# wsakobe/CylinderTag

Measured on AMD Instinct MI355X. Metric: frames/sec detect() 1920x1080, higher is better.
Workload: dtype u8; 1 GPU; synthetic 1920x1080 random-stripe frames, 4096 per step over 1 GPU(s), 4 planted CTag_2f12c markers each, detect(img,5,true,5), inputs resident in HBM; frames_per_gpu=4096, chunk=4096, parallelism=frames sharded, dp1, gather=none (1 GPU)

## Files before the change

### cylindertag_amd/csrc/ctag_api.hip

```cpp
#include <hip/hip_runtime.h>

#include <algorithm>
#include <climits>
#include <cmath>
#include <cstdio>
#include <cstdlib>
#include <cstring>
#include <fstream>
#include <map>
#include <mutex>
#include <new>
#include <string>
#include <type_traits>
#include <vector>

#include "../../include/ctag.h"
#include "ctag_internal.h"

using namespace ctag;

#define HIP_TRY(expr)                                                                                   \
    do {                                                                                                \
        hipError_t e__ = (expr);                                                                        \
        if (e__ != hipSuccess) {                                                                        \
// ... 262 lines not shown
    put(W.xmin, pool);
    put(W.ymin, pool);
    put(W.xmax, pool);
    put(W.ymax, pool);
    put(W.key, pool);
    put(W.pool_tile, pool);
    put(W.member_head, pool);
    put(W.member_next, pool);
    put(W.ncand, F * 4);
    put(W.nroots, F * 4);
    put(W.cand, F * CC * sizeof(Candidate));
    put(W.quads, F * CC * sizeof(QuadOut));
    put(W.line_count, F * 4);
    put(W.clp_used, F * 4);
    put(W.line_long, F * 4);
    put(W.cl_pool, F * (size_t)W.cl_cap * 4 + 16);
    put(W.line_desc, F * LC * sizeof(LineDesc));
    put(W.line_sorted, F * LC * 4);
    put(W.line_fit, F * LC * 16);
    put(W.cand_aux, F * CC * sizeof(CandAux));
    put(W.npacks, F * 8);
    put(W.packs, F * CC * 4);
    put(W.pack_order, F * CC * 4);
    put(W.welsch_rs, std::min<size_t>(F, kLatencyFrames) * kLatLines * 20 * 6 * 4);
    put(W.quad_derived, F * kQuadStride * 48);
    put(W.quad_index, F * kQuadStride * 4);
    put(W.nquads, F * 4);
    put(W.nfeat, F * 4);
    put(W.status, F * 4);
    put(W.feat0, F * CTAG_MAX_FEATURES * sizeof(FeatureDev));
    put(W.feat1, F * CTAG_MAX_FEATURES * sizeof(FeatureDev));
    put(W.feat2, F * CTAG_MAX_FEATURES * sizeof(FeatureDev));
    put(W.premarkers, F * sizeof(ctag_frame_result));
    put(W.frame_long, F * 4);
    put(W.rz_xofs, (size_t)g.hcols * 4);
    put(W.rz_alpha, (size_t)g.hcols * 8);
    put(W.rz_yofs, (size_t)g.hrows * 4);
    put(W.rz_beta, (size_t)g.hrows * 8);
    return off;
}

static int ensure_workspace(ctag_handle* h, ctag_handle::WsSlot& S, int rows, int cols, int tw, int frames, bool big, bool need_n0) {
    auto refresh = [&](Workspace& W) {
        const Caps c = make_caps(make_geom(rows, cols, tw, h->params.area_max_fraction), h->params, big);
        W.g = make_geom(rows, cols, tw, h->params.area_max_fraction);
        W.g.pool_cap = c.pool_cap;
// ... 1025 lines not shown
```

### cylindertag_amd/csrc/ctag_internal.h

```cpp
#pragma once
#include <hip/hip_runtime.h>
#include <stddef.h>
#include <stdint.h>

#include <vector>

#include "../../include/ctag_types.h"

struct ctag_handle;
struct ctag_camera;
struct ctag_pose_rec;
struct ctag_rig_pose_rec;
struct ctag_mv_pose_rec;
struct ctag_camera_set;

namespace ctag {
template <class T>
struct DevBuf {
    T* p = nullptr;
    size_t cap = 0;
    DevBuf() = default;
    DevBuf(const DevBuf&) = delete;
    DevBuf& operator=(const DevBuf&) = delete;
    ~DevBuf() { release(); }
// ... 152 lines not shown
    int32_t* key = nullptr;
    int32_t* pool_tile = nullptr;
    int32_t* member_head = nullptr;
    int32_t* member_next = nullptr;
    int32_t* ncand = nullptr;
    int32_t* nroots = nullptr;
    int cand_cap = 0;
    int line_cap = 0;
    uint32_t cl_cap = 0;
    bool big = false;
    Candidate* cand = nullptr;
    QuadOut* quads = nullptr;
    int32_t* line_count = nullptr;
    int32_t* clp_used = nullptr;
    uint32_t* cl_pool = nullptr;
    LineDesc* line_desc = nullptr;
    int32_t* line_sorted = nullptr;
    int32_t* line_long = nullptr;
    float* line_fit = nullptr;
    CandAux* cand_aux = nullptr;
    int32_t* npacks = nullptr;
    uint32_t* packs = nullptr;
    uint32_t* pack_order = nullptr;
    float* welsch_rs = nullptr;
    const uint8_t* pick_table = nullptr;
    const uint16_t* pick_table16 = nullptr;
    hipStream_t aux_stream = nullptr;
    hipEvent_t ev_fork = nullptr, ev_join = nullptr;
    KParams kp{};
    void* quad_derived = nullptr;
    int32_t* quad_index = nullptr;
    int32_t* nquads = nullptr;
    int32_t* nfeat = nullptr;
    int32_t* status = nullptr;
    FeatureDev* feat0 = nullptr;
    FeatureDev* feat1 = nullptr;
    FeatureDev* feat2 = nullptr;
    ctag_frame_result* premarkers = nullptr;
    double* refine_n0 = nullptr;
    int32_t* frame_long = nullptr;
    int32_t* rz_xofs = nullptr;
    int16_t* rz_alpha = nullptr;
    int32_t* rz_yofs = nullptr;
    int16_t* rz_beta = nullptr;
    void* base = nullptr;
    size_t bytes = 0;
// ... 161 lines not shown
```

### cylindertag_amd/csrc/k_quad.hip

```cpp
#include "ctag_internal.h"
#include "ctag_math.h"
#include "ctag_wave.h"
#include <cstdio>
#include <type_traits>
#include <cstdlib>

namespace ctag {

struct QuadPtrs {
    const uint16_t* labels;
    const int32_t* tile_base;
    const int32_t* root_of;
    const int32_t* ncand;
    const Candidate* cand;
    QuadOut* quads;
    uint32_t* frame_flags;
    int32_t* line_count;
    int32_t* clp_used;
    uint32_t* cl_pool;
    LineDesc* line_desc;
    int32_t* line_sorted;
    int32_t* line_long;
    float* line_fit;
    CandAux* cand_aux;
    const uint8_t* pick_table;
    const uint16_t* pick_table16;
    const int32_t* pool_tile;
    const int32_t* member_head;
    const int32_t* member_next;
    int32_t* npacks;
    uint32_t* packs;
    uint32_t* pack_order;
    unsigned long long* stamps;
    float thr_line, thr_expand, rac;
    int c2_far, c2_near;
    int cand_cap, line_cap;
    uint32_t cl_cap;
    float expand_eps;
    const uint64_t* mask;
    int mask_words;
};
static QuadPtrs quad_ptrs(const ChunkPlan& pl, const Workspace& ws, unsigned long long* stamps) {
    QuadPtrs P{};
    P.labels = ws.labels, P.tile_base = ws.tile_base, P.root_of = ws.root_of, P.ncand = ws.ncand, P.cand = ws.cand, P.quads = ws.quads, P.frame_flags = ws.frame_flags;
    P.line_count = ws.line_count, P.clp_used = ws.clp_used, P.cl_pool = ws.cl_pool, P.line_desc = ws.line_desc, P.line_sorted = ws.line_sorted, P.line_long = ws.line_long;
    P.line_fit = ws.line_fit, P.cand_aux = ws.cand_aux, P.pick_table = ws.pick_table, P.pick_table16 = ws.pick_table16;
    P.pool_tile = ws.pool_tile, P.member_head = ws.member_head, P.member_next = ws.member_next;
    P.npacks = ws.npacks, P.packs = ws.packs, P.pack_order = ws.pack_order, P.stamps = stamps;
    P.thr_line = ws.kp.thr_line, P.thr_expand = ws.kp.thr_expand, P.rac = ws.kp.rac, P.c2_far = ws.kp.c2_far, P.c2_near = ws.kp.c2_near, P.expand_eps = ws.kp.expand_eps;
    P.cand_cap = ws.cand_cap, P.line_cap = ws.line_cap, P.cl_cap = ws.cl_cap;
    P.mask = pl.fused ? reinterpret_cast<const uint64_t*>(ws.half) : nullptr, P.mask_words = ws.g.hcols >> 6;
    return P;
}

__device__ __forceinline__ uint32_t pack_xy(int x, int y) { return (uint32_t)x | ((uint32_t)y << 16); }
__device__ __forceinline__ int ux(uint32_t p) { return (int)(p & 0xffffu); }
__device__ __forceinline__ int uy(uint32_t p) { return (int)(p >> 16); }

__device__ __forceinline__ void moments_to_line(double x, double y, double x2, double y2, double xy, double w, float* line) {
    const ctm::Recip64 W = ctm::recip64(w);
    x = ctm::div64(x, W);
    y = ctm::div64(y, W);
    x2 = ctm::div64(x2, W);
    y2 = ctm::div64(y2, W);
    xy = ctm::div64(xy, W);
    const double dx2 = x2 - x * x, dy2 = y2 - y * y, dxy = xy - x * y;
    const float t = (float)ctm::atan2_64(2 * dxy, dx2 - dy2) / 2;
    double sn, cs;
    ctm::sincos64(t, &sn, &cs);
    line[0] = (float)cs;
    line[1] = (float)sn;
// ... 217 lines not shown
    (void)welsch_rounds<WS, COUNT>(pts, n, EPS, line, err, 0, 30, false, wc, min(n, kWCap), trips);
    restart_store(res, rstride, line, err);
}

#ifndef CTAG_PACK_WORDS
#define CTAG_PACK_WORDS 5120
#endif
#ifndef CTAG_PACK_WAVES
#define CTAG_PACK_WAVES 2
#endif
constexpr int kPackWords = CTAG_PACK_WORDS;
#ifndef CTAG_PACK_WAVES_P2
#define CTAG_PACK_WAVES_P2 4
#endif
constexpr int kPackWordsSmall = 2560, kPackWavesSmall = 4, kPackWavesSmallP2 = CTAG_PACK_WAVES_P2;
constexpr int kUnwind = 8;
constexpr int kWaveWords = 8192;
constexpr int kWaveWordsMax = 36864;
__host__ __device__ __forceinline__ int pack_points(int w, int h) { return min(2 * (w + h), w * h) + 1; }
__host__ __device__ __forceinline__ int pack_need(int w, int h) {
    const int C = pack_points(w, h);
    return ((w + 1) & ~1) + 2 * h + 2 * C + 4;
}
constexpr int kScanWords = 2048;
__host__ __device__ __forceinline__ int scan_need(int w, int h) { return w + 3 * h + 4; }
constexpr int kMaskScanWords = 512, kMaskScanWordsLarge = 2048;
__host__ __device__ __forceinline__ int mask_scan_need(int w, int h) { return h * ((w + 31) / 32 + 1); }
__host__ __device__ __forceinline__ bool pack_big(int x_min, int w, int h, int big_points, int pack_words, int scan_words = 0) {
    (void)x_min;
    return pack_need(w, h) > pack_words || pack_points(w, h) > big_points || (scan_words > 0 && scan_need(w, h) > scan_words) ||
           (scan_words < 0 && mask_scan_need(w, h) > -scan_words);
}

struct CornerPre {
    float x, y, dis, ang;
};

__global__ __launch_bounds__(1024) void k_pack(QuadPtrs P, int nframes, int max_per_pack, int big_points, int pack_words, int scan_words) {
    __shared__ int s_key[kLdsCand + 2];
    __shared__ int s_need[kLdsCand];
    __shared__ uint16_t s_ord[kLdsCand];
    const int frame = blockIdx.x;
    if (frame >= nframes) return;
    const int tid = threadIdx.x, nt = blockDim.x;
    const int nc = min(P.ncand[frame], P.cand_cap);
    const Candidate* cand = P.cand + (size_t)frame * P.cand_cap;
    uint32_t* order = P.pack_order + (size_t)frame * P.cand_cap;
    uint32_t* packs = P.packs + (size_t)frame * P.cand_cap;
    auto key_of = [&](const Candidate& c) {
        const int w = c.x_max - c.x_min + 1, h = c.y_max - c.y_min + 1;
        return pack_big(c.x_min, w, h, big_points, pack_words, scan_words) ? -1 : pack_points(w, h);
    };
    auto build_packs = [&](int npacked, auto need_of) {
        int np = 0, first = -1, cnt = 0, words = 0;
        for (int r0 = 0; r0 < npacked; r0 += 64) {
            const int r = r0 + tid;
            const int need = r < npacked ? need_of(r) : 0;
            const int m = min(64, npacked - r0);
            for (int k = 0; k < m; k++) {
                const int nk = __builtin_amdgcn_readlane(need, k);
                if (cnt > 0 && (cnt == max_per_pack || words + nk > pack_words)) {
                    if (tid == 0) packs[np] = (uint32_t)first | ((uint32_t)cnt << 24);
                    np++;
                    cnt = 0;
                    words = 0;
                }
                if (cnt == 0) first = r0 + k;
                cnt++;
                words += nk;
            }
        }
        if (cnt > 0) {
            if (tid == 0) packs[np] = (uint32_t)first | ((uint32_t)cnt << 24);
            np++;
        }
        return np;
    };
    auto slot_prefix = [&](int npacked, auto ci_of) {
        int base = 0;
        for (int r0 = 0; r0 < npacked; r0 += 64) {
            const int r = r0 + tid;
            int v = 0, ci = 0;
            if (r < npacked) {
                ci = ci_of(r);
                const Candidate c = cand[ci];
                v = pack_points(c.x_max - c.x_min + 1, c.y_max - c.y_min + 1) + 64;
            }
            int incl = v;
#pragma unroll
            for (int d = 1; d < 64; d <<= 1) {
                const int t = __shfl_up(incl, d, 64);
                if (tid >= d) incl += t;
            }
            if (r < npacked) P.cand_aux[(size_t)frame * P.cand_cap + ci].line0 = base + incl - v;
            base += __shfl(incl, 63, 64);
        }
        if (tid == 0) P.clp_used[frame] = base;
    };
    if (nc > kLdsCand) {
        constexpr int kB = kLdsCand;
        auto bucket_of = [&](int key) { return key < 0 ? kB : kB - 1 - min(key, kB - 1); };
        for (int b = tid; b <= kB; b += nt) s_key[b] = 0;
        __syncthreads();
        for (int i = tid; i < nc; i += nt) atomicAdd(&s_key[bucket_of(key_of(cand[i]))], 1);
        __syncthreads();
        if (tid == 0) {
            int run = 0;
            for (int b = 0; b <= kB; b++) {
                const int v = s_key[b];
                s_key[b] = run;
                run += v;
            }
            s_key[kB + 1] = run;
        }
        __syncthreads();
        const int first_big = s_key[kB];
        __syncthreads();
        for (int i = tid; i < nc; i += nt) order[atomicAdd(&s_key[bucket_of(key_of(cand[i]))], 1)] = (uint32_t)i;
        __syncthreads();
        if (tid >= 64) return;
        const int np = build_packs(first_big, [&](int r) {
            const Candidate c = cand[order[r]];
            return pack_need(c.x_max - c.x_min + 1, c.y_max - c.y_min + 1);
        });
        if (tid == 0) {
            P.npacks[2 * frame] = np;
            P.npacks[2 * frame + 1] = nc - first_big;
        }
        if (scan_words < 0) slot_prefix(first_big, [&](int r) { return (int)order[r]; });
        return;
    }
    for (int i = tid; i < nc; i += nt) {
        const Candidate c = cand[i];
        const int w = c.x_max - c.x_min + 1, h = c.y_max - c.y_min + 1;
        s_key[i] = key_of(c);
        s_need[i] = pack_need(w, h);
    }
    if (tid == 0) s_key[kLdsCand] = 0;
    __syncthreads();
    for (int i = tid; i < nc; i += nt) {
        const int ki = s_key[i];
        int rank = 0;
        for (int j = 0; j < nc; j++) {
            const int kj = s_key[j];
            rank += (kj > ki || (kj == ki && j < i)) ? 1 : 0;
        }
        s_ord[rank] = (uint16_t)i;
        if (ki < 0) atomicAdd(&s_key[kLdsCand], 1);
    }
    __syncthreads();
    for (int i = tid; i < nc; i += nt) order[i] = s_ord[i];
    if (tid >= 64) return;
    const int nbig = s_key[kLdsCand];
    const int np = build_packs(nc - nbig, [&](int r) { return s_need[s_ord[r]]; });
    if (tid == 0) {
        P.npacks[2 * frame] = np;
        P.npacks[2 * frame + 1] = nbig;
    }
    if (scan_words < 0) slot_prefix(nc - nbig, [&](int r) { return (int)s_ord[r]; });
}


#ifndef CTAG_EXPAND_INLINE
#define CTAG_EXPAND_INLINE __forceinline__
#endif
struct ALine {
    double c, s, x, y;
    bool ok;
};
__device__ __forceinline__ ALine approx_line(long long sx, long long sy, long long sxx, long long syy, long long sxy, int cnt, double k2lim) {
    const double n = (double)cnt, fx = (double)sx, fy = (double)sy;
    const double rn = __builtin_amdgcn_rcp(n);
    const double A = ((double)sxx * n - fx * fx) - ((double)syy * n - fy * fy);
    const double B = 2.0 * ((double)sxy * n - fx * fy);
    const double h2 = A * A + B * B;
    const double rh = __builtin_amdgcn_rsq(h2);
    const double u = ctm::fabs64(A) * rh;
    const double p = 0.5 + 0.5 * u;
    const double rp = __builtin_amdgcn_rsq(p);
    const double big = p * rp, small = (0.5 * ctm::fabs64(B) * rh) * rp;
    const bool bneg = B < 0.0;
    ALine L;
// ... 368 lines not shown
                aux->acx = 0.f;
                aux->acy = 0.f;
                aux->n_boundary = 0;
            }
        }
    }
}

template <int SG, int WORDS, int WAVES, bool DYN, bool REFPRM, int PHASE = 0, bool PRESCAN = false>
__global__ __launch_bounds__(64) __attribute__((amdgpu_waves_per_eu(WAVES, WAVES))) void k_quad_edges_packed(QuadPtrs P, FrameGeom g, int nframes, int tier_lo) {
    static_assert(PHASE != 3 || (SG == 64 && !PRESCAN), "the scan-only build is a whole-wave build");
    static_assert(!PRESCAN || (SG == 8 && PHASE != 2), "PRESCAN: a packed build that would otherwise scan");
    const float k_thr_line = REFPRM ? 1.8f : P.thr_line, k_thr_expand = REFPRM ? 1.2f : P.thr_expand;
    const int k_c2_far = REFPRM ? 2 : P.c2_far, k_c2_near = REFPRM ? 1 : P.c2_near;
    static_assert(SG == 8 || SG == 64, "8 lanes per component (packs) or the whole wave (oversize components)");
    __shared__ uint32_t s_static[DYN ? 1 : WORDS];
    extern __shared__ uint32_t s_dynamic[];
    uint32_t* const s_mem = DYN ? s_dynamic : s_static;
    const int frame = blockIdx.x;
    if (frame >= nframes) return;
    const int lane = threadIdx.x, sub = lane / SG, sl = lane % SG, lane0 = lane - sl;
    const int nc = min(P.ncand[frame], P.cand_cap);
    const int npk = PHASE == 3 ? nc - P.npacks[2 * frame + 1]
                               : P.npacks[2 * frame + (SG == 8 ? 0 : 1)];
    const uint16_t* __restrict__ limg = P.labels + ((size_t)frame * g.hrows) * g.lp;
    const int32_t* __restrict__ tbase = P.tile_base + (size_t)frame * g.tiles_x * g.tiles_y;
    const int32_t* __restrict__ rootof = P.root_of + (size_t)frame * g.pool_cap;

    unsigned long long t_prev = 0;
    auto stamp = [&](int phase) {
        if (P.stamps) {
            const unsigned long long t = __builtin_amdgcn_s_memtime();
            if (phase >= 0 && lane == 0) atomicAdd(&P.stamps[phase + (SG == 64 ? 8 : 0)], t - t_prev);
            t_prev = t;
        }
    };
    for (int pk = blockIdx.y; pk < npk; pk += gridDim.y) {
        __syncthreads();
        stamp(-1);
        int first, cnt;
        if constexpr (SG == 8) {
            const uint32_t pw = P.packs[(size_t)frame * P.cand_cap + pk];
            first = (int)(pw & 0xffffffu);
            cnt = (int)(pw >> 24);
        } else if constexpr (PHASE == 3) {
            first = pk;
            cnt = 1;
        } else {
            first = nc - npk + pk;
            cnt = 1;
        }
        const bool act = sub < cnt;
        const int ci = (int)P.pack_order[(size_t)frame * P.cand_cap + first + (act ? sub : 0)];
        const Candidate cd = P.cand[(size_t)frame * P.cand_cap + ci];
        const int x_min = cd.x_min, y_min = cd.y_min;
        const int w = cd.x_max - cd.x_min + 1, h = cd.y_max - cd.y_min + 1;
        const int C = pack_points(w, h);
        const int need = act ? (PHASE == 3 ? scan_need(w, h) : pack_need(w, h)) : 0;
        int off = 0;
#pragma unroll
        for (int k = 0; k < 64 / SG; k++) {
            const int v = __shfl(need, k * SG);
            if (k < sub) off += v;
        }
        if (!act) continue;
        CandAux* aux = P.cand_aux + (size_t)frame * P.cand_cap + ci;
        if constexpr (SG == 64 && PHASE != 3) {
            if (need <= tier_lo) continue;
            if (need > WORDS) {
                if (tier_lo > 0 && sl == 0) {
                    atomicOr(&P.frame_flags[frame], CTAG_FLAG_POOL_OVERFLOW);
                    aux->line0 = -1;
                    aux->acx = 0.f;
                    aux->acy = 0.f;
                    aux->n_boundary = 0;
                }
                continue;
            }
        }
        uint32_t* mem = s_mem + off;
        uint32_t* tb = mem;
        uint32_t* lr = tb + w + 2;
        uint32_t* bufA = lr + h + 2;
        uint32_t* bufB = bufA + (PHASE == 3 ? h : C);
        uint32_t* lef = bufA;
        uint32_t* rig = bufB;
        const int sgshift = sub * SG;

        int n = 0, n_boundary = 0, p0 = 0;
        float acx = 0.f, acy = 0.f;
        if constexpr (PHASE != 2 && !PRESCAN) {
        stamp(6);
#ifndef CTAG_KEYS_LARGE
#define CTAG_KEYS_LARGE 16
#endif
#ifndef CTAG_KEYS_SMALL
#define CTAG_KEYS_SMALL 8
#endif
        constexpr int kMaxKeys = (SG == 8 && WORDS > kPackWordsSmall) ? CTAG_KEYS_LARGE : CTAG_KEYS_SMALL;
        uint32_t mykey[kMaxKeys];
        bool many = false;
        {
            const int32_t* ptile = P.pool_tile + (size_t)frame * g.pool_cap;
            const int32_t* mnext = P.member_next + (size_t)frame * g.pool_cap;
            int e = cd.root;
            bool first_e = true;
#pragma unroll
// ... 704 lines not shown
                aux->line0 = -1;
                aux->acx = 0.f;
                aux->acy = 0.f;
                aux->n_boundary = n_boundary;
            }
            continue;
        }
        }
        }
        if constexpr (PHASE == 1) {
            uint32_t* slot = P.cl_pool + (size_t)frame * P.cl_cap + p0;
            for (int k = sl; k < n; k += SG) slot[k] = bufB[k];
            if (sl == 0) {
                aux->line0 = p0;
                aux->acx = acx;
                aux->acy = acy;
                aux->n_boundary = n_boundary;
            }
            continue;
        }
        if constexpr (PHASE == 2) {
            p0 = aux->line0;
            if (p0 < 0) continue;
            n = n_boundary = aux->n_boundary;
            acx = aux->acx;
            acy = aux->acy;
            const uint32_t* slot = P.cl_pool + (size_t)frame * P.cl_cap + p0;
            for (int k = sl; k < n; k += SG) bufB[k] = slot[k];
            wave_fence();
        }
        uint32_t* CLg = P.cl_pool + (size_t)frame * P.cl_cap + p0;
        uint32_t* W = bufB;
        uint32_t* Wn = bufA;
        int cnt_b = 0, init = 0, cl_off[5] = {0, 0, 0, 0, 0};
        bool failed = false;
        unsigned long long rdp_t = 0, rdp_acc[4] = {0, 0, 0, 0}, exp_dbg[3] = {0, 0, 0};
        auto rdp_mark = [&](int slot) {
            if (SG == 64 && P.stamps) {
                const unsigned long long t = __builtin_amdgcn_s_memtime();
                if (slot >= 0) rdp_acc[slot] += t - rdp_t;
                rdp_t = t;
            }
        };
        rdp_mark(-1);
        while (n > 0 && !failed && cnt_b < 4) {
            auto tri2 = [&](int a) {
                const uint32_t q0 = W[a], q2 = W[(a + 2) % n], q1 = W[(a + 1) % n];
                const int vx = ux(q0) + ux(q2) - 2 * ux(q1), vy = uy(q0) + uy(q2) - 2 * uy(q1);
                return vx * vx + vy * vy;
// ... 103 lines not shown
        bool ok = true;
        for (int j = 0; j < 4; j++) {
            const int len = (j < cnt_b) ? (cl_off[j + 1] - cl_off[j]) : 0;
            if (len < 2) ok = false;
        }
        if (cl_off[min(cnt_b, 4)] >= C + 64) ok = false;
        int l0 = -1;
        if (ok) {
            if (sl == 0) l0 = atomicAdd(&P.line_count[frame], 4);
            l0 = __shfl(l0, lane0);
            if (l0 + 4 > P.line_cap) {
                ok = false;
                if (sl == 0) atomicOr(&P.frame_flags[frame], CTAG_FLAG_POOL_OVERFLOW);
            }
        }
        if (ok && sl < 4) {
            LineDesc d;
            d.off = (uint32_t)(p0 + cl_off[sl]);
            d.n = cl_off[sl + 1] - cl_off[sl];
            P.line_desc[(size_t)frame * P.line_cap + l0 + sl] = d;
        }
        if (sl == 0) {
            aux->line0 = ok ? l0 : -1;
            aux->acx = ok ? acx : 0.f;
            aux->acy = ok ? acy : 0.f;
            aux->n_boundary = n_boundary;
        }
        stamp(4);
    }
}

constexpr int kWShort = 10;
constexpr int kLineSortBuckets = 2048;
constexpr int kLineSortThreads = 1024;
__global__ __launch_bounds__(kLineSortThreads) void k_line_sort(QuadPtrs P, int nframes) {
    __shared__ int s_n[kLdsLines];
    __shared__ int s_long;
    const int frame = blockIdx.x;
    if (frame >= nframes) return;
    const int L = min(P.line_count[frame], P.line_cap);
    const LineDesc* d = P.line_desc + (size_t)frame * P.line_cap;
    int32_t* out = P.line_sorted + (size_t)frame * P.line_cap;
    if (threadIdx.x == 0) s_long = 0;
    __syncthreads();
    if (L > kLdsLines) {
        constexpr int kB = kLineSortBuckets;
        static_assert(kB - 1 > kLatPoints && kB + 1 <= kLdsLines, "shared bucket");
        auto bucket_of = [&](int n) { return kB - 1 - min(n, kB - 1); };
        for (int b = threadIdx.x; b <= kB; b += kLineSortThreads) s_n[b] = 0;
// ... 651 lines not shown
#pragma unroll
    for (int j = 0; j < 4; j++) {
        out->c[2 * j] = valid ? bc[j].x : 0.f;
        out->c[2 * j + 1] = valid ? bc[j].y : 0.f;
    }
}

#ifndef CTAG_SCAN_WAVES
#define CTAG_SCAN_WAVES 4
#endif
template <bool REF>
static void launch_quad_edges(const ChunkPlan& pl, const QuadPtrs& P, const FrameGeom& g, hipStream_t s, hipStream_t sb, hipStream_t s_max, hipEvent_t mid) {
    const int nframes = pl.nframes;
    const dim3 grid(nframes, pl.pack_gx);
    if (pl.all_wave) {
    } else if (pl.prescan) {
        if (pl.mask_scan)
            if (pl.small_cfg) hipLaunchKernelGGL((k_silhouette_mask<4, 32, kMaskScanWords>), dim3(nframes, pl.mscan_gx), dim3(64), 0, s, P, g, nframes);
            else hipLaunchKernelGGL((k_silhouette_mask<8, 64, kMaskScanWordsLarge>), dim3(nframes, 2 * pl.mscan_gx), dim3(64), 0, s, P, g, nframes);
        else
            hipLaunchKernelGGL((k_quad_edges_packed<64, kScanWords, CTAG_SCAN_WAVES, false, true, 3>), dim3(nframes, pl.scan_gx), dim3(64), 0, s, P, g, nframes, 0);
        if (pl.small_cfg) {
            hipLaunchKernelGGL((k_quad_edges_packed<8, kPackWordsSmall, kPackWavesSmall, false, REF, 1, true>), grid, dim3(64), 0, s, P, g, nframes, 0);
            hipLaunchKernelGGL((k_quad_edges_packed<8, kPackWordsSmall, kPackWavesSmallP2, false, REF, 2>), grid, dim3(64), 0, s, P, g, nframes, 0);
        } else {
            hipLaunchKernelGGL((k_quad_edges_packed<8, kPackWords, CTAG_PACK_WAVES, false, REF, 0, true>), grid, dim3(64), 0, s, P, g, nframes, 0);
        }
    } else if (pl.small_cfg) {
        hipLaunchKernelGGL((k_quad_edges_packed<8, kPackWordsSmall, kPackWavesSmall, false, REF, 1>), grid, dim3(64), 0, s, P, g, nframes, 0);
        hipLaunchKernelGGL((k_quad_edges_packed<8, kPackWordsSmall, kPackWavesSmallP2, false, REF, 2>), grid, dim3(64), 0, s, P, g, nframes, 0);
    } else {
        hipLaunchKernelGGL((k_quad_edges_packed<8, kPackWords, CTAG_PACK_WAVES, false, REF>), grid, dim3(64), 0, s, P, g, nframes, 0);
    }
    if (mid) (void)hipEventRecord(mid, s);
    ensure_dynamic_lds(reinterpret_cast<const void*>(&k_quad_edges_packed<64, kWaveWordsMax, 1, true, REF>), kWaveWordsMax * 4);
    hipLaunchKernelGGL((k_quad_edges_packed<64, kWaveWords, 1, false, REF>), dim3(nframes, pl.big_cols), dim3(64), 0, sb, P, g, nframes, 0);
    hipLaunchKernelGGL((k_quad_edges_packed<64, kWaveWordsMax, 1, true, REF>), dim3(nframes, pl.big_max_gx), dim3(64), kWaveWordsMax * 4, s_max, P, g, nframes, kWaveWords);
}

hipError_t launch_line_fits(const ChunkPlan& pl, const Workspace& ws, hipStream_t s, unsigned long long* stamps, hipEvent_t ev_sorted) {
    const int nframes = pl.nframes;
    const QuadPtrs P = quad_ptrs(pl, ws, stamps);
    hipLaunchKernelGGL(k_line_sort, dim3(nframes), dim3(kLineSortThreads), 0, s, P, nframes);
    if (ev_sorted) (void)hipEventRecord(ev_sorted, s);
    const bool welsch_lat = pl.latency && ws.welsch_rs;
    if (welsch_lat) {
        hipLaunchKernelGGL(k_welsch_lat, dim3(20, kLatRankBlocks, nframes), dim3(64), 0, s, P, nframes, ws.welsch_rs);
    }
    hipLaunchKernelGGL(stamps ? k_welsch<true> : k_welsch<false>, dim3(nframes, pl.welsch_gx + pl.welsch_gs), dim3(kWT), 0, s, P, nframes, welsch_lat ? ws.welsch_rs : (const float*)nullptr, pl.welsch_gx);
    return hipPeekAtLastError();
}

// ... 96 lines not shown
```

### include/ctag_testkit.h

```cpp
#ifndef CTAG_TESTKIT_H
#define CTAG_TESTKIT_H
#include <stddef.h>
#include <stdint.h>

#include "ctag.h"
#include "ctag_pose.h"

#ifdef __cplusplus
extern "C" {
#endif

#define CTAG_DBG_HALF 1
#define CTAG_DBG_LABELS 2
#define CTAG_DBG_CANDIDATES 3
#define CTAG_DBG_CAND_QUADS 4
#define CTAG_DBG_FEATURES0 5
#define CTAG_DBG_FEATURES1 6
#define CTAG_DBG_FEATURES2 7
#define CTAG_DBG_PREMARKERS 8
#define CTAG_DBG_GRAY 9
#define CTAG_DBG_MASK 11
#define CTAG_DBG_LINES 10
#define CTAG_DBG_LINE_POINTS 12
#define CTAG_DBG_LINE_FITS 13
long ctag_debug_fetch(ctag_handle* h, int frame, int what, void* dst, size_t capacity_elems);

int ctag_math_probe(ctag_handle* h, int op, int n, const double* a, const double* b, double* out);

int ctag_testkit_exp32_k0_sweep(uint32_t first_bits, uint32_t last_bits, uint32_t step, uint64_t* counts, uint32_t* first_bad);

int ctag_testkit_unpack_gathered(ctag_handle* h, const void* gathered_dev, int n_total, int world, uint64_t width,
                                 ctag_frame_result* out_dev);

int ctag_testkit_stall_stream(ctag_handle* h, int milliseconds);

typedef struct ctag_synth_truth {
    int32_t n_markers;
    int32_t dict_row[8];
    float strip_len[8];
    float corners[8][8];
} ctag_synth_truth;
int ctag_synth_frames_device(ctag_handle* h, uint8_t* frames_dev, int first_frame, int n, int rows, int cols,
                             ptrdiff_t row_stride, ptrdiff_t frame_stride, uint64_t seed, int markers_per_frame);
int ctag_synth_frame_host(const int32_t* state, int dict_rows, int dict_cols, uint8_t* frame, int frame_index, int rows,
                          int cols, ptrdiff_t row_stride, uint64_t seed, int markers_per_frame, ctag_synth_truth* truth);
int ctag_synth_layout_truth(const int32_t* state, int dict_rows, int dict_cols, int frame_index, int rows, int cols, uint64_t seed,
                            int markers_per_frame, ctag_synth_truth* truth);
// ... 55 lines not shown
```

### testkit/__init__.py

```python
import ctypes as C
import os
import subprocess

import numpy as np

import cylindertag_amd as ca
from cylindertag_amd import capi
from cylindertag_amd.capi import CtagError, Model

_HERE = os.path.dirname(os.path.abspath(__file__))
_LIB = os.environ.get("CTAG_TESTKIT_LIB") or os.path.join(_HERE, "_build", "libctag_testkit.so")

TRUTH3D_DT = np.dtype([("n_markers", "<i4"), ("dict_row", "<i4", (8,)), ("_pad", "<i4", (1,)), ("R", "<f8", (8, 9)), ("t", "<f8", (8, 3)),
                       ("radius", "<f8", (8,))])
TRUTH_DT = np.dtype([("n_markers", "<i4"), ("dict_row", "<i4", (8,)), ("strip_len", "<f4", (8,)),
                     ("corners", "<f4", (8, 8))])
DBG_HALF, DBG_LABELS, DBG_CANDIDATES, DBG_CAND_QUADS, DBG_FEATURES0, DBG_FEATURES1, DBG_FEATURES2, DBG_PREMARKERS, DBG_GRAY, DBG_LINES, DBG_MASK, DBG_LINE_POINTS, DBG_LINE_FITS = range(1, 14)
SYNTH_SEED = 0x4354616753594E00

EXPORTS = ["ctag_debug_fetch", "ctag_math_probe", "ctag_testkit_exp32_k0_sweep", "ctag_testkit_unpack_gathered", "ctag_testkit_stall_stream", "ctag_synth_frames_device", "ctag_synth_frame_host",
           "ctag_synth_layout_truth", "ctag_synth3d_frames_device", "ctag_synth3d_frame_host", "ctag_synth3d_model",
           "ctag_testkit_dense_edge_probe", "ctag_testkit_plan", "ctag_testkit_welsch_fit", "ctag_testkit_welsch_limits",
           "ctag_testkit_model_fit_system", "ctag_testkit_model_fit_limits", "ctag_testkit_rig_fit_system", "ctag_testkit_rig_fit_limits",
           "ctag_testkit_camera_fit_system", "ctag_testkit_camera_fit_limits",
           "ctag_testkit_intrinsics_fit_system", "ctag_testkit_intrinsics_fit_poses", "ctag_testkit_intrinsics_fit_limits"]
PLAN_FIELDS = ("fused", "bgr_direct", "zero_first", "dec_zero_kernel", "dec_zero_list", "dec", "dec_xblocks", "dec_yblocks", "dec_band_rows", "dec_bands",
               "ccl", "latency", "small_cfg", "refprm", "mask_scan", "prescan", "all_wave", "fork", "pack_max", "big_points", "pack_gx", "scan_gx",
               "mscan_gx", "big_cols", "big_max_gx", "welsch_gs", "welsch_gx", "refine", "refine_gx", "refine_sums_gx")
DEC_FORMS = ("mask", "mask_bands", "general", "wide", "banded135", "banded", "unaligned")
CCL_FORMS = ("mask", "tw5", "any")
WELSCH_LIMITS = ("kWShort", "kWCap", "kWRes", "kWPts", "kWPtsU", "kPickN", "kPickN2", "kWE", "kWT", "kLatLines", "kLatPoints", "kLatChunk", "kLdsLines",
                 "kLatencyFrames", "kLatRankBlocks", "kLineSortBuckets")
REFINE_FORMS = ("none", "one", "split_large", "split_looping", "split")
MATH_EXP32_NONPOS, MATH_EXP32_NONPOS_K0 = 15, 17


def lib_path():
    return _LIB


# ... 200 lines not shown
            raise CtagError(st, "ctag_synth_frames_device")

    def synth3d_frames_device(self, frames_ptr, first, n, rows, cols, row_stride, frame_stride, K, seed=SYNTH_SEED, markers=4):
        K = np.asarray(K, np.float64)
        st = self.T.ctag_synth3d_frames_device(self.h, frames_ptr, first, n, rows, cols, row_stride, frame_stride, seed, markers,
                                               K[0, 0], K[1, 1], K[0, 2], K[1, 2])
        if st != 0:
            raise CtagError(st, "ctag_synth3d_frames_device")

    def stall_stream(self, milliseconds):
        st = self.T.ctag_testkit_stall_stream(self.h, int(milliseconds))
        if st != 0:
            raise CtagError(st, "ctag_testkit_stall_stream")

    def unpack_gathered(self, gathered_ptr, n_total, world, width, out_ptr):
        self._gcheck(self.T.ctag_testkit_unpack_gathered(self.h, gathered_ptr, n_total, world, width, out_ptr), "ctag_testkit_unpack_gathered")

    def debug(self, frame, what):
        n = self.T.ctag_debug_fetch(self.h, frame, what, None, 0)
        if n < 0:
            raise CtagError(-1, "ctag_debug_fetch(%d)" % what)
        if what in (DBG_HALF, DBG_GRAY, DBG_MASK):
            a = np.zeros(n, np.uint8)
        elif what in (DBG_LABELS, DBG_CANDIDATES, DBG_LINES, DBG_LINE_POINTS):
            a = np.zeros(n, np.int32)
        elif what == DBG_PREMARKERS:
            a = np.zeros(1, ca.RESULT_DT)
        else:
            a = np.zeros(n, np.float32)
        if n:
            got = self.T.ctag_debug_fetch(self.h, frame, what, a.ctypes.data, max(n, 1))
            if got < 0:
                raise CtagError(-2, "ctag_debug_fetch(%d)" % what)
        if what in (DBG_CANDIDATES, DBG_CAND_QUADS):
            return a.reshape(-1, 8)
        if what in (DBG_FEATURES0, DBG_FEATURES1, DBG_FEATURES2):
            return a.reshape(-1, 19)
        if what == DBG_PREMARKERS:
            return a[0]
        if what == DBG_LINE_POINTS:
            return a.reshape(-1, 2)
        if what == DBG_LINE_FITS:
            return a.reshape(-1, 4)
        return a

    def welsch_fit(self, frames, latency=0, welsch_gx=0, welsch_gs=0, tail_at_pool_end=False):
        clusters = [np.asarray(c, np.int32).reshape(-1, 2) for f in frames for c in f]
# ... 109 lines not shown
```

### testkit/ctag_testkit.hip

```cpp
#include <hip/hip_runtime.h>

#include <algorithm>
#include <cstring>
#include <vector>

#include "../include/ctag_testkit.h"
#include "../cylindertag_amd/csrc/ctag_internal.h"
#include "../cylindertag_amd/csrc/ctag_math.h"
#include "ctag_synth.h"

using namespace ctag;

#define TK_TRY(expr)                              \
    do {                                          \
        if ((expr) != hipSuccess) return CTAG_ERR_HIP; \
    } while (0)

namespace {

__global__ void k_math_probe(int op, int n, const double* a, const double* b, double* out) {
    const int i = blockIdx.x * blockDim.x + threadIdx.x;
    if (i >= n) return;
    const double x = a[i], y = b[i];
    double r = 0;
// ... 345 lines not shown
            if (nl > 0 && !d2h(d.data(), W.line_desc + (size_t)frame * W.line_cap, sizeof(LineDesc) * nl)) return -2;
            if (what == CTAG_DBG_LINE_FITS) {
                if (dst && cap >= (size_t)nl * 4 && nl > 0 && !d2h(dst, W.line_fit + (size_t)frame * W.line_cap * 4, (size_t)nl * 16)) return -2;
                return (long)nl * 4;
            }
            size_t total = 0, extent = 0;
            for (int i = 0; i < nl; i++) {
                if (d[i].n < 0 || (size_t)d[i].off + (size_t)d[i].n > (size_t)W.cl_cap) return -2;
                total += (size_t)d[i].n;
                extent = std::max(extent, (size_t)d[i].off + (size_t)d[i].n);
            }
            if (dst && cap >= total * 2 && total > 0) {
                std::vector<uint32_t> pool(extent);
                if (!d2h(pool.data(), W.cl_pool + (size_t)frame * W.cl_cap, extent * 4)) return -2;
                int32_t* o = static_cast<int32_t*>(dst);
                for (int i = 0; i < nl; i++)
                    for (int j = 0; j < d[i].n; j++) {
                        const uint32_t w = pool[(size_t)d[i].off + j];
                        *o++ = (int32_t)(w & 0xffffu);
                        *o++ = (int32_t)(w >> 16);
                    }
            }
            return (long)(total * 2);
        }
        case CTAG_DBG_PREMARKERS: {
            if (!v.keep_pre) return -1;
            if (dst && cap >= 1) {
                if (!d2h(dst, W.premarkers + frame, sizeof(ctag_frame_result))) return -2;
            }
            return 1;
        }
        default: return -1;
    }
}

int ctag_math_probe(ctag_handle* h, int op, int n, const double* a, const double* b, double* out) {
    if (!h || n < 0 || !a || !out) return CTAG_ERR_ARG;
    if (n == 0) return CTAG_OK;
    HandleView v{};
    handle_view(h, &v);
    TK_TRY(hipSetDevice(v.device));
    hipStream_t s = static_cast<hipStream_t>(ctag_stream(h));
    double *da = nullptr, *db = nullptr, *dout = nullptr;
    int rc = CTAG_OK;
    if (hipMalloc(reinterpret_cast<void**>(&da), (size_t)n * 8) != hipSuccess || hipMalloc(reinterpret_cast<void**>(&db), (size_t)n * 8) != hipSuccess ||
        hipMalloc(reinterpret_cast<void**>(&dout), (size_t)n * 8) != hipSuccess)
// ... 295 lines not shown
```

Baseline: 268,300 frames/s.

## Repack phase-2 quad edge work by boundary size between phase kernels

Adds a k_repack kernel that runs after phase 1 of the small-config packed quad-edge pass. It re-sorts only the surviving candidates (valid line0, non-zero boundary) by their boundary point count and builds new packs sized to the actual phase-2 need instead of the phase-1 bounding-box need. Phase 2 then reads the new pack list and order, compacts its LDS layout to two buffers, and skips rewriting acx/acy/n_boundary. The intent is to drop dead candidates and fit more work per wave in phase 2, at the cost of an extra kernel launch per chunk and additional workspace buffers.

Result: faster. 275,900 frames/s (median of 6 runs) (+2.9%).

```diff
diff --git a/cylindertag_amd/csrc/ctag_api.hip b/cylindertag_amd/csrc/ctag_api.hip
--- a/cylindertag_amd/csrc/ctag_api.hip
+++ b/cylindertag_amd/csrc/ctag_api.hip
@@ -308,6 +308,9 @@
     put(W.npacks, F * 8);
     put(W.packs, F * CC * 4);
     put(W.pack_order, F * CC * 4);
+    put(W.npacks2, F * 8);
+    put(W.packs2, F * CC * 4);
+    put(W.pack_order2, F * CC * 4);
     put(W.welsch_rs, std::min<size_t>(F, kLatencyFrames) * kLatLines * 20 * 6 * 4);
     put(W.quad_derived, F * kQuadStride * 48);
     put(W.quad_index, F * kQuadStride * 4);
diff --git a/cylindertag_amd/csrc/ctag_internal.h b/cylindertag_amd/csrc/ctag_internal.h
--- a/cylindertag_amd/csrc/ctag_internal.h
+++ b/cylindertag_amd/csrc/ctag_internal.h
@@ -198,6 +198,9 @@
     int32_t* npacks = nullptr;
     uint32_t* packs = nullptr;
     uint32_t* pack_order = nullptr;
+    int32_t* npacks2 = nullptr;
+    uint32_t* packs2 = nullptr;
+    uint32_t* pack_order2 = nullptr;
     float* welsch_rs = nullptr;
     const uint8_t* pick_table = nullptr;
     const uint16_t* pick_table16 = nullptr;
diff --git a/cylindertag_amd/csrc/k_quad.hip b/cylindertag_amd/csrc/k_quad.hip
--- a/cylindertag_amd/csrc/k_quad.hip
+++ b/cylindertag_amd/csrc/k_quad.hip
@@ -31,6 +31,9 @@
     int32_t* npacks;
     uint32_t* packs;
     uint32_t* pack_order;
+    int32_t* npacks2;
+    uint32_t* packs2;
+    uint32_t* pack_order2;
     unsigned long long* stamps;
     float thr_line, thr_expand, rac;
     int c2_far, c2_near;
@@ -47,6 +50,7 @@
     P.line_fit = ws.line_fit, P.cand_aux = ws.cand_aux, P.pick_table = ws.pick_table, P.pick_table16 = ws.pick_table16;
     P.pool_tile = ws.pool_tile, P.member_head = ws.member_head, P.member_next = ws.member_next;
     P.npacks = ws.npacks, P.packs = ws.packs, P.pack_order = ws.pack_order, P.stamps = stamps;
+    P.npacks2 = ws.npacks2, P.packs2 = ws.packs2, P.pack_order2 = ws.pack_order2;
     P.thr_line = ws.kp.thr_line, P.thr_expand = ws.kp.thr_expand, P.rac = ws.kp.rac, P.c2_far = ws.kp.c2_far, P.c2_near = ws.kp.c2_near, P.expand_eps = ws.kp.expand_eps;
     P.cand_cap = ws.cand_cap, P.line_cap = ws.line_cap, P.cl_cap = ws.cl_cap;
     P.mask = pl.fused ? reinterpret_cast<const uint64_t*>(ws.half) : nullptr, P.mask_words = ws.g.hcols >> 6;
@@ -310,6 +314,7 @@
     const int C = pack_points(w, h);
     return ((w + 1) & ~1) + 2 * h + 2 * C + 4;
 }
+__host__ __device__ __forceinline__ int need2(int n) { return 2 * ((n + 1) & ~1); }
 constexpr int kScanWords = 2048;
 __host__ __device__ __forceinline__ int scan_need(int w, int h) { return w + 3 * h + 4; }
 constexpr int kMaskScanWords = 512, kMaskScanWordsLarge = 2048;
@@ -323,6 +328,71 @@
 struct CornerPre {
     float x, y, dis, ang;
 };
+
+__device__ __forceinline__ int pack_rank_sort(const int* s_key, uint16_t* s_ord, int n, int tid, int nt) {
+    int neg = 0;
+    for (int i = tid; i < n; i += nt) {
+        const int ki = s_key[i];
+        int rank = 0;
+        for (int j = 0; j < n; j++) {
+            const int kj = s_key[j];
+            rank += (kj > ki || (kj == ki && j < i)) ? 1 : 0;
+        }
+        s_ord[rank] = (uint16_t)i;
+        neg += ki < 0 ? 1 : 0;
+    }
+    return neg;
+}
+template <class KeyOf, class ValOf>
+__device__ __forceinline__ int pack_counting_sort(int* s_cnt, uint32_t* out, int n, int tid, int nt, KeyOf key_of, ValOf val_of) {
+    constexpr int kB = kLdsCand;
+    auto bucket_of = [&](int key) { return key < 0 ? kB : kB - 1 - min(key, kB - 1); };
+    for (int b = tid; b <= kB; b += nt) s_cnt[b] = 0;
+    __syncthreads();
+    for (int i = tid; i < n; i += nt) atomicAdd(&s_cnt[bucket_of(key_of(i))], 1);
+    __syncthreads();
+    if (tid == 0) {
+        int run = 0;
+        for (int b = 0; b <= kB; b++) {
+            const int v = s_cnt[b];
+            s_cnt[b] = run;
+            run += v;
+        }
+        s_cnt[kB + 1] = run;
+    }
+    __syncthreads();
+    const int first_neg = s_cnt[kB];
+    __syncthreads();
+    for (int i = tid; i < n; i += nt) out[atomicAdd(&s_cnt[bucket_of(key_of(i))], 1)] = val_of(i);
+    __syncthreads();
+    return first_neg;
+}
+template <class NeedOf>
+__device__ __forceinline__ int build_packs(uint32_t* packs, int npacked, int max_per_pack, int pack_words, int tid, NeedOf need_of) {
+    int np = 0, first = -1, cnt = 0, words = 0;
+    for (int r0 = 0; r0 < npacked; r0 += 64) {
+        const int r = r0 + tid;
+        const int need = r < npacked ? need_of(r) : 0;
+        const int m = min(64, npacked - r0);
+        for (int k = 0; k < m; k++) {
+            const int nk = __builtin_amdgcn_readlane(need, k);
+            if (cnt > 0 && (cnt == max_per_pack || words + nk > pack_words)) {
+                if (tid == 0) packs[np] = (uint32_t)first | ((uint32_t)cnt << 24);
+                np++;
+                cnt = 0;
+                words = 0;
+            }
+            if (cnt == 0) first = r0 + k;
+            cnt++;
+            words += nk;
+        }
+    }
+    if (cnt > 0) {
+        if (tid == 0) packs[np] = (uint32_t)first | ((uint32_t)cnt << 24);
+        np++;
+    }
+    return np;
+}
 
 __global__ __launch_bounds__(1024) void k_pack(QuadPtrs P, int nframes, int max_per_pack, int big_points, int pack_words, int scan_words) {
     __shared__ int s_key[kLdsCand + 2];
@@ -339,31 +409,6 @@
         const int w = c.x_max - c.x_min + 1, h = c.y_max - c.y_min + 1;
         return pack_big(c.x_min, w, h, big_points, pack_words, scan_words) ? -1 : pack_points(w, h);
     };
-    auto build_packs = [&](int npacked, auto need_of) {
-        int np = 0, first = -1, cnt = 0, words = 0;
-        for (int r0 = 0; r0 < npacked; r0 += 64) {
-            const int r = r0 + tid;
-            const int need = r < npacked ? need_of(r) : 0;
-            const int m = min(64, npacked - r0);
-            for (int k = 0; k < m; k++) {
-                const int nk = __builtin_amdgcn_readlane(need, k);
-                if (cnt > 0 && (cnt == max_per_pack || words + nk > pack_words)) {
-                    if (tid == 0) packs[np] = (uint32_t)first | ((uint32_t)cnt << 24);
-                    np++;
-                    cnt = 0;
-                    words = 0;
-                }
-                if (cnt == 0) first = r0 + k;
-                cnt++;
-                words += nk;
-            }
-        }
-        if (cnt > 0) {
-            if (tid == 0) packs[np] = (uint32_t)first | ((uint32_t)cnt << 24);
-            np++;
-        }
-        return np;
-    };
     auto slot_prefix = [&](int npacked, auto ci_of) {
         int base = 0;
         for (int r0 = 0; r0 < npacked; r0 += 64) {
@@ -386,28 +431,9 @@
         if (tid == 0) P.clp_used[frame] = base;
     };
     if (nc > kLdsCand) {
-        constexpr int kB = kLdsCand;
-        auto bucket_of = [&](int key) { return key < 0 ? kB : kB - 1 - min(key, kB - 1); };
-        for (int b = tid; b <= kB; b += nt) s_key[b] = 0;
-        __syncthreads();
-        for (int i = tid; i < nc; i += nt) atomicAdd(&s_key[bucket_of(key_of(cand[i]))], 1);
-        __syncthreads();
-        if (tid == 0) {
-            int run = 0;
-            for (int b = 0; b <= kB; b++) {
-                const int v = s_key[b];
-                s_key[b] = run;
-                run += v;
-            }
-            s_key[kB + 1] = run;
-        }
-        __syncthreads();
-        const int first_big = s_key[kB];
-        __syncthreads();
-        for (int i = tid; i < nc; i += nt) order[atomicAdd(&s_key[bucket_of(key_of(cand[i]))], 1)] = (uint32_t)i;
-        __syncthreads();
+        const int first_big = pack_counting_sort(s_key, order, nc, tid, nt, [&](int i) { return key_of(cand[i]); }, [&](int i) { return (uint32_t)i; });
         if (tid >= 64) return;
-        const int np = build_packs(first_big, [&](int r) {
+        const int np = build_packs(packs, first_big, max_per_pack, pack_words, tid, [&](int r) {
             const Candidate c = cand[order[r]];
             return pack_need(c.x_max - c.x_min + 1, c.y_max - c.y_min + 1);
         });
@@ -426,26 +452,53 @@
     }
     if (tid == 0) s_key[kLdsCand] = 0;
     __syncthreads();
-    for (int i = tid; i < nc; i += nt) {
-        const int ki = s_key[i];
-        int rank = 0;
-        for (int j = 0; j < nc; j++) {
-            const int kj = s_key[j];
-            rank += (kj > ki || (kj == ki && j < i)) ? 1 : 0;
-        }
-        s_ord[rank] = (uint16_t)i;
-        if (ki < 0) atomicAdd(&s_key[kLdsCand], 1);
-    }
+    if (const int neg = pack_rank_sort(s_key, s_ord, nc, tid, nt)) atomicAdd(&s_key[kLdsCand], neg);
     __syncthreads();
     for (int i = tid; i < nc; i += nt) order[i] = s_ord[i];
     if (tid >= 64) return;
     const int nbig = s_key[kLdsCand];
-    const int np = build_packs(nc - nbig, [&](int r) { return s_need[s_ord[r]]; });
+    const int np = build_packs(packs, nc - nbig, max_per_pack, pack_words, tid, [&](int r) { return s_need[s_ord[r]]; });
     if (tid == 0) {
         P.npacks[2 * frame] = np;
         P.npacks[2 * frame + 1] = nbig;
     }
     if (scan_words < 0) slot_prefix(nc - nbig, [&](int r) { return (int)s_ord[r]; });
+}
+
+__global__ __launch_bounds__(64) void k_repack(QuadPtrs P, int nframes, int max_per_pack, int pack_words) {
+    __shared__ int s_key[kLdsCand + 2];
+    __shared__ uint16_t s_ord[kLdsCand];
+    const int frame = blockIdx.x;
+    if (frame >= nframes) return;
+    const int tid = threadIdx.x, nt = blockDim.x;
+    const int nc = min(P.ncand[frame], P.cand_cap);
+    const int npk = max(nc - P.npacks[2 * frame + 1], 0);
+    const CandAux* aux = P.cand_aux + (size_t)frame * P.cand_cap;
+    const uint32_t* order = P.pack_order + (size_t)frame * P.cand_cap;
+    uint32_t* order2 = P.pack_order2 + (size_t)frame * P.cand_cap;
+    uint32_t* packs2 = P.packs2 + (size_t)frame * P.cand_cap;
+    auto key_of = [&](int r) {
+        const CandAux a = aux[order[r]];
+        return (a.line0 >= 0 && a.n_boundary > 0) ? a.n_boundary : -1;
+    };
+    int nel, np;
+    if (npk > kLdsCand) {
+        nel = pack_counting_sort(s_key, order2, npk, tid, nt, key_of, [&](int r) { return order[r]; });
+        np = build_packs(packs2, nel, max_per_pack, pack_words, tid, [&](int r) { return need2(aux[order2[r]].n_boundary); });
+    } else {
+        for (int r = tid; r < npk; r += nt) s_key[r] = key_of(r);
+        if (tid == 0) s_key[kLdsCand] = 0;
+        __syncthreads();
+        if (const int neg = pack_rank_sort(s_key, s_ord, npk, tid, nt)) atomicAdd(&s_key[kLdsCand], neg);
+        __syncthreads();
+        nel = npk - s_key[kLdsCand];
+        for (int i = tid; i < nel; i += nt) order2[i] = order[s_ord[i]];
+        np = build_packs(packs2, nel, max_per_pack, pack_words, tid, [&](int r) { return need2(s_key[s_ord[r]]); });
+    }
+    if (tid == 0) {
+        P.npacks2[2 * frame] = np;
+        P.npacks2[2 * frame + 1] = nel;
+    }
 }
 
 
@@ -860,7 +913,11 @@
     const int lane = threadIdx.x, sub = lane / SG, sl = lane % SG, lane0 = lane - sl;
     const int nc = min(P.ncand[frame], P.cand_cap);
     const int npk = PHASE == 3 ? nc - P.npacks[2 * frame + 1]
+                  : PHASE == 2 ? P.npacks2[2 * frame]
                                : P.npacks[2 * frame + (SG == 8 ? 0 : 1)];
+    static_assert(PHASE != 2 || SG == 8, "the second kernel is a packed build");
+    const uint32_t* __restrict__ pack_list = (PHASE == 2 ? P.packs2 : P.packs) + (size_t)frame * P.cand_cap;
+    const uint32_t* __restrict__ pack_ord = (PHASE == 2 ? P.pack_order2 : P.pack_order) + (size_t)frame * P.cand_cap;
     const uint16_t* __restrict__ limg = P.labels + ((size_t)frame * g.hrows) * g.lp;
     const int32_t* __restrict__ tbase = P.tile_base + (size_t)frame * g.tiles_x * g.tiles_y;
     const int32_t* __restrict__ rootof = P.root_of + (size_t)frame * g.pool_cap;
@@ -878,7 +935,7 @@
         stamp(-1);
         int first, cnt;
         if constexpr (SG == 8) {
-            const uint32_t pw = P.packs[(size_t)frame * P.cand_cap + pk];
+            const uint32_t pw = pack_list[pk];
             first = (int)(pw & 0xffffffu);
             cnt = (int)(pw >> 24);
         } else if constexpr (PHASE == 3) {
@@ -889,12 +946,15 @@
             cnt = 1;
         }
         const bool act = sub < cnt;
-        const int ci = (int)P.pack_order[(size_t)frame * P.cand_cap + first + (act ? sub : 0)];
+        const int ci = (int)pack_ord[first + (act ? sub : 0)];
         const Candidate cd = P.cand[(size_t)frame * P.cand_cap + ci];
+        CandAux* aux = P.cand_aux + (size_t)frame * P.cand_cap + ci;
         const int x_min = cd.x_min, y_min = cd.y_min;
         const int w = cd.x_max - cd.x_min + 1, h = cd.y_max - cd.y_min + 1;
         const int C = pack_points(w, h);
-        const int need = act ? (PHASE == 3 ? scan_need(w, h) : pack_need(w, h)) : 0;
+        int nb2 = 0;
+        if constexpr (PHASE == 2) nb2 = aux->n_boundary;
+        const int need = act ? (PHASE == 3 ? scan_need(w, h) : PHASE == 2 ? need2(nb2) : pack_need(w, h)) : 0;
         int off = 0;
 #pragma unroll
         for (int k = 0; k < 64 / SG; k++) {
@@ -902,7 +962,6 @@
             if (k < sub) off += v;
         }
         if (!act) continue;
-        CandAux* aux = P.cand_aux + (size_t)frame * P.cand_cap + ci;
         if constexpr (SG == 64 && PHASE != 3) {
             if (need <= tier_lo) continue;
             if (need > WORDS) {
@@ -919,8 +978,8 @@
         uint32_t* mem = s_mem + off;
         uint32_t* tb = mem;
         uint32_t* lr = tb + w + 2;
-        uint32_t* bufA = lr + h + 2;
-        uint32_t* bufB = bufA + (PHASE == 3 ? h : C);
+        uint32_t* bufA = PHASE == 2 ? mem + (need >> 1) : lr + h + 2;
+        uint32_t* bufB = PHASE == 2 ? mem : bufA + (PHASE == 3 ? h : C);
         uint32_t* lef = bufA;
         uint32_t* rig = bufB;
         const int sgshift = sub * SG;
@@ -1671,9 +1730,7 @@
         if constexpr (PHASE == 2) {
             p0 = aux->line0;
             if (p0 < 0) continue;
-            n = n_boundary = aux->n_boundary;
-            acx = aux->acx;
-            acy = aux->acy;
+            n = nb2;
             const uint32_t* slot = P.cl_pool + (size_t)frame * P.cl_cap + p0;
             for (int k = sl; k < n; k += SG) bufB[k] = slot[k];
             wave_fence();
@@ -1823,9 +1880,13 @@
         }
         if (sl == 0) {
             aux->line0 = ok ? l0 : -1;
-            aux->acx = ok ? acx : 0.f;
-            aux->acy = ok ? acy : 0.f;
-            aux->n_boundary = n_boundary;
+            if constexpr (PHASE == 2) {
+                if (!ok) aux->acx = 0.f, aux->acy = 0.f;
+            } else {
+                aux->acx = ok ? acx : 0.f;
+                aux->acy = ok ? acy : 0.f;
+                aux->n_boundary = n_boundary;
+            }
         }
         stamp(4);
     }
@@ -2523,12 +2584,14 @@
             hipLaunchKernelGGL((k_quad_edges_packed<64, kScanWords, CTAG_SCAN_WAVES, false, true, 3>), dim3(nframes, pl.scan_gx), dim3(64), 0, s, P, g, nframes, 0);
         if (pl.small_cfg) {
             hipLaunchKernelGGL((k_quad_edges_packed<8, kPackWordsSmall, kPackWavesSmall, false, REF, 1, true>), grid, dim3(64), 0, s, P, g, nframes, 0);
+            hipLaunchKernelGGL(k_repack, dim3(nframes), dim3(64), 0, s, P, nframes, pl.pack_max, kPackWordsSmall);
             hipLaunchKernelGGL((k_quad_edges_packed<8, kPackWordsSmall, kPackWavesSmallP2, false, REF, 2>), grid, dim3(64), 0, s, P, g, nframes, 0);
         } else {
             hipLaunchKernelGGL((k_quad_edges_packed<8, kPackWords, CTAG_PACK_WAVES, false, REF, 0, true>), grid, dim3(64), 0, s, P, g, nframes, 0);
         }
     } else if (pl.small_cfg) {
         hipLaunchKernelGGL((k_quad_edges_packed<8, kPackWordsSmall, kPackWavesSmall, false, REF, 1>), grid, dim3(64), 0, s, P, g, nframes, 0);
+        hipLaunchKernelGGL(k_repack, dim3(nframes), dim3(64), 0, s, P, nframes, pl.pack_max, kPackWordsSmall);
         hipLaunchKernelGGL((k_quad_edges_packed<8, kPackWordsSmall, kPackWavesSmallP2, false, REF, 2>), grid, dim3(64), 0, s, P, g, nframes, 0);
     } else {
         hipLaunchKernelGGL((k_quad_edges_packed<8, kPackWords, CTAG_PACK_WAVES, false, REF>), grid, dim3(64), 0, s, P, g, nframes, 0);
diff --git a/include/ctag_testkit.h b/include/ctag_testkit.h
--- a/include/ctag_testkit.h
+++ b/include/ctag_testkit.h
@@ -23,6 +23,7 @@
 #define CTAG_DBG_LINES 10
 #define CTAG_DBG_LINE_POINTS 12
 #define CTAG_DBG_LINE_FITS 13
+#define CTAG_DBG_PACKS 14
 long ctag_debug_fetch(ctag_handle* h, int frame, int what, void* dst, size_t capacity_elems);
 
 int ctag_math_probe(ctag_handle* h, int op, int n, const double* a, const double* b, double* out);
diff --git a/testkit/__init__.py b/testkit/__init__.py
--- a/testkit/__init__.py
+++ b/testkit/__init__.py
@@ -15,7 +15,7 @@
                        ("radius", "<f8", (8,))])
 TRUTH_DT = np.dtype([("n_markers", "<i4"), ("dict_row", "<i4", (8,)), ("strip_len", "<f4", (8,)),
                      ("corners", "<f4", (8, 8))])
-DBG_HALF, DBG_LABELS, DBG_CANDIDATES, DBG_CAND_QUADS, DBG_FEATURES0, DBG_FEATURES1, DBG_FEATURES2, DBG_PREMARKERS, DBG_GRAY, DBG_LINES, DBG_MASK, DBG_LINE_POINTS, DBG_LINE_FITS = range(1, 14)
+DBG_HALF, DBG_LABELS, DBG_CANDIDATES, DBG_CAND_QUADS, DBG_FEATURES0, DBG_FEATURES1, DBG_FEATURES2, DBG_PREMARKERS, DBG_GRAY, DBG_LINES, DBG_MASK, DBG_LINE_POINTS, DBG_LINE_FITS, DBG_PACKS = range(1, 15)
 SYNTH_SEED = 0x4354616753594E00
 
 EXPORTS = ["ctag_debug_fetch", "ctag_math_probe", "ctag_testkit_exp32_k0_sweep", "ctag_testkit_unpack_gathered", "ctag_testkit_stall_stream", "ctag_synth_frames_device", "ctag_synth_frame_host",
@@ -262,7 +262,7 @@
             raise CtagError(-1, "ctag_debug_fetch(%d)" % what)
         if what in (DBG_HALF, DBG_GRAY, DBG_MASK):
             a = np.zeros(n, np.uint8)
-        elif what in (DBG_LABELS, DBG_CANDIDATES, DBG_LINES, DBG_LINE_POINTS):
+        elif what in (DBG_LABELS, DBG_CANDIDATES, DBG_LINES, DBG_LINE_POINTS, DBG_PACKS):
             a = np.zeros(n, np.int32)
         elif what == DBG_PREMARKERS:
             a = np.zeros(1, ca.RESULT_DT)
diff --git a/testkit/ctag_testkit.hip b/testkit/ctag_testkit.hip
--- a/testkit/ctag_testkit.hip
+++ b/testkit/ctag_testkit.hip
@@ -391,6 +391,32 @@
                     }
             }
             return (long)(total * 2);
+        }
+        case CTAG_DBG_PACKS: {
+            int32_t hd[5] = {0, 0, 0, 0, 0};
+            if (!d2h(&hd[0], W.ncand + frame, 4) || !d2h(&hd[1], W.npacks + 2 * frame, 8) || !d2h(&hd[3], W.npacks2 + 2 * frame, 8)) return -2;
+            hd[0] = std::min(hd[0], W.cand_cap);
+            const size_t nc = (size_t)hd[0], np1 = (size_t)hd[1], np2 = (size_t)hd[3], nel = (size_t)hd[4];
+            if (hd[1] < 0 || hd[3] < 0 || hd[4] < 0 || np1 > nc || np2 > nc || nel > nc) return -2;
+            const size_t total = 5 + np1 + np2 + nc + nel + nc;
+            if (dst && cap >= total) {
+                int32_t* o = static_cast<int32_t*>(dst);
+                std::memcpy(o, hd, sizeof(hd));
+                o += 5;
+                const size_t fo = (size_t)frame * W.cand_cap;
+                if (np1 && !d2h(o, W.packs + fo, np1 * 4)) return -2;
+                o += np1;
+                if (np2 && !d2h(o, W.packs2 + fo, np2 * 4)) return -2;
+                o += np2;
+                if (nc && !d2h(o, W.pack_order + fo, nc * 4)) return -2;
+                o += nc;
+                if (nel && !d2h(o, W.pack_order2 + fo, nel * 4)) return -2;
+                o += nel;
+                std::vector<CandAux> a(std::max<size_t>(nc, 1));
+                if (nc && !d2h(a.data(), W.cand_aux + fo, nc * sizeof(CandAux))) return -2;
+                for (size_t i = 0; i < nc; i++) o[i] = a[i].n_boundary;
+            }
+            return (long)total;
         }
         case CTAG_DBG_PREMARKERS: {
             if (!v.keep_pre) return -1;
```
